# han0110/learn-fhe

Measured on AMD Instinct MI355X. Metric: NTTs/sec at N=2^14 q~60-bit, higher is better.
Workload: dtype u64

## Files before the change

learn-fhe_amd/csrc/arith.hpp:

```cpp
#pragma once
#include <type_traits>

#include "dev_arith.hpp"

namespace fhe {

#define FHE_GLOBAL __attribute__((address_space(1)))
template <class T>
__device__ __forceinline__ const FHE_GLOBAL T *as_global(const T *p) {
    return (const FHE_GLOBAL T *)p;
}
#define FHE_CONST __attribute__((address_space(4)))
template <class T>
__device__ __forceinline__ const FHE_CONST T *as_const(const T *p) {
    return (const FHE_CONST T *)p;
}

#define FHE_HEADER_KERNEL static __attribute__((unused)) __global__

template <int I, int END, typename F>
__device__ __forceinline__ void static_for(F &&f) {
    if constexpr (I < END) {
        f(std::integral_constant<int, I>{});
        static_for<I + 1, END>(f);
// ... 92 lines not shown
    static __device__ __forceinline__ u64 mac_in(u64 x, const K &k) { return canon4(x, k.q, k.q2); }
    static __device__ __forceinline__ u64 mac(u64 acc, u64 xin, u64 kval, int, const K &k, const Barrett &B) {
        return csub(acc + mulmod_barrett(xin, kval, B), k.q);
    }
    static __device__ __forceinline__ u64 mac_finish(u64 acc, const K &) { return acc; }
};

struct PmTw {
    unsigned wl, wlp, wh;
};
typedef uint2 PmRaw;
struct PmK {
    u64 q, q2, q4;
    unsigned c, c2;
};

__device__ __forceinline__ u64 mad_u64(unsigned a, unsigned b, u64 c) {
    u64 d, carry;
    asm("v_mad_u64_u32 %0, %1, %2, %3, %4" : "=v"(d), "=s"(carry) : "v"(a), "v"(b), "v"(c));
    return d;
}

__device__ __forceinline__ u64 hi_word(u64 x) {
    u64 d;
    asm("v_lshrrev_b64 %0, 32, %1" : "=v"(d) : "v"(x));
    return d;
}

template <int B>
__device__ __forceinline__ void pm_mul_vu(u64 y, const PmTw w, u64 &v, u64 &u) {
    const unsigned y0 = (unsigned)y, y1 = (unsigned)(y >> 32);
    const u64 z0 = (u64)w.wl * y0;
    const u64 z1 = (u64)w.wh * y0 + (u64)w.wlp * y1;
    v = mad_u64((unsigned)z1, 1u << (B - 31), z0);
    u = (u64)w.wh * y1 + hi_word(z1);
}

template <int B>
__device__ __forceinline__ u64 pm_reduce_vu(u64 v, u64 u, const PmK &k) {
    constexpr unsigned HMASK = (1u << (B - 32)) - 1;
    const u64 r1 = (u64)(unsigned)u * k.c2 + v;
    const u64 r2 = (u64)(unsigned)(u >> 32) * k.c2 + (r1 >> 32);
    const unsigned h2 = (unsigned)(r2 >> (B - 32));
    const u64 l2 = ((u64)((unsigned)r2 & HMASK) << 32) | (unsigned)r1;
    return (u64)h2 * k.c + l2;
}

template <int B>
__device__ __forceinline__ u64 pm_mul(u64 y, const PmTw w, const PmK &k) {
    u64 v, u;
    pm_mul_vu<B>(y, w, v, u);
    return pm_reduce_vu<B>(v, u, k);
}

template <int B>
struct ArithPM {
    typedef u64 Elem;
    static constexpr u64 MASK = (u64(1) << B) - 1;
    struct K {
        PmK m;
        const FHE_CONST PmRaw *tw, *twi;
        PmTw ninv;
        PmTw ninv_w;
        int pb, prefix;
    };
    typedef PmRaw TwRaw;
    typedef PmTw TwReg;
    static constexpr int PREFETCH = 4;
    static __host__ __device__ __forceinline__ u64 pack(u64 w) { return ((w >> (B - 31)) << 32) | (w & ((u64(1) << (B - 31)) - 1)); }
    template <bool INV>
    static __device__ __forceinline__ TwRaw fetch(const K &k, int idx) {
        const FHE_CONST PmRaw *p = (INV ? k.twi : k.tw) + idx;
        TwRaw r;
        r.x = p->x; r.y = p->y;
        return r;
    }
    static __device__ __forceinline__ TwReg prep(const TwRaw &r) { return PmTw{r.x, r.x << (63 - B), r.y}; }
    static __host__ __device__ __forceinline__ PmTw split(u64 w) {
        PmTw t;
        t.wl = (unsigned)(w & ((u64(1) << (B - 31)) - 1));
        t.wlp = t.wl << (63 - B);
        t.wh = (unsigned)(w >> (B - 31));
        return t;
    }
    static __device__ __forceinline__ K make(const ModDesc &D, int log_n_total, int pb, int prefix) {
        K k;
        k.m.q = D.q; k.m.q2 = 2 * D.q; k.m.q4 = 4 * D.q;
        k.m.c = D.pm_c; k.m.c2 = 2 * D.pm_c;
        k.tw = (const FHE_CONST PmRaw *)D.tww; k.twi = (const FHE_CONST PmRaw *)D.twwi;
        k.ninv = split(pb ? 1 : D.ninv[log_n_total]);
        k.ninv_w = split(D.ninv_w[log_n_total]);
        k.pb = pb; k.prefix = prefix;
        return k;
    }
    static __device__ __forceinline__ u64 fold1(u64 x, const PmK &m) {
        const unsigned hi = (unsigned)(x >> 32), h = hi >> (B - 32);
        const u64 base = ((u64)(hi & (unsigned)(MASK >> 32)) << 32) | (unsigned)x;
        return (u64)h * m.c + base;
    }
    static __device__ __forceinline__ u64 mulvar(u64 x, u64 y, const K &k) { return pm_mul<B>(x, split(y), k.m); }
    static __device__ __forceinline__ void ct(u64 &X, u64 &Y, const TwReg &w, const K &k) {
        const u64 t = pm_mul<B>(Y, w, k.m);
        const u64 x = X;
        X = x + t;
        Y = x - t + k.m.q2;
    }
    template <int PH>
    static __device__ __forceinline__ void gs(u64 &X, u64 &Y, const TwReg &w, const K &k) {
        const u64 s = X + Y;
        const u64 d = X - Y + (PH ? k.m.q4 : k.m.q2);
        X = s;
        Y = pm_mul<B>(d, w, k.m);
    }
    static constexpr bool GS_FOLDS = true;
    static constexpr int GS_SPAN = 0;
    template <int PH = 1>
    static __device__ __forceinline__ void gs_last_scaled(u64 &X, u64 &Y, const K &k) {
        const u64 s = X + Y, d = X - Y + k.m.q4;
        X = csub(pm_mul<B>(s, k.ninv, k.m), k.m.q);
        Y = csub(pm_mul<B>(d, k.ninv_w, k.m), k.m.q);
    }
    template <int PH = 1>
    static __device__ __forceinline__ void gs_last_plain(u64 &X, u64 &Y, const PmTw &w, const K &k) {
        const u64 s = X + Y, d = X - Y + k.m.q4;
        X = csub(fold1(s, k.m), k.m.q);
        Y = csub(pm_mul<B>(d, w, k.m), k.m.q);
    }
    static constexpr int CT_LAYERS = ((1 << (63 - B)) + 1) / 2 > 64 ? 64 : ((1 << (63 - B)) + 1) / 2;
    static constexpr bool PASS_FOLD = true;
    static __device__ constexpr bool ct_fold_at(int) { return false; }
    static __device__ __forceinline__ u64 gs_fold(u64 x, const K &k) { return fold1(x, k.m); }
    static __device__ __forceinline__ u64 fold(u64 x, const K &k) { return fold1(x, k.m); }
    static __device__ __forceinline__ u64 canon_fwd(u64 x, const K &k) { return csub(fold1(x, k.m), k.m.q); }
    static __device__ __forceinline__ u64 finish_inv(u64 x, const K &k) { return csub(pm_mul<B>(x, k.ninv, k.m), k.m.q); }
    static constexpr int MAC_TERMS = B <= 54 ? 32 : B == 55 ? 16 : B == 56 ? 8 : 3;
    struct MacAcc { u64 v, u; };
    static __device__ __forceinline__ MacAcc mac_zero() { return MacAcc{0, 0}; }
    static __device__ __forceinline__ u64 mac_in(u64 x, const K &) { return x; }
    static __device__ __forceinline__ MacAcc mac(MacAcc acc, u64 xin, u64 kval, int term, const K &k, const Barrett &) {
        const unsigned wl = (unsigned)kval;
        const PmTw w{wl, wl << (63 - B), (unsigned)(kval >> 32)};
        u64 v, u;
        pm_mul_vu<B>(xin, w, v, u);
        acc.v += v; acc.u += u;
        if ((term % MAC_TERMS) == MAC_TERMS - 1) acc = MacAcc{pm_reduce_vu<B>(acc.v, acc.u, k.m), 0};
        return acc;
    }
    static __device__ __forceinline__ u64 mac_finish(MacAcc acc, const K &k) { return pm_reduce_vu<B>(acc.v, acc.u, k.m); }
};

struct DsK {
    u64 q, q2, q4;
    unsigned c, c2, pw;
};

template <int B>
struct ArithDS {
    typedef u64 Elem;
    static constexpr u64 MASK = (u64(1) << B) - 1;
    static constexpr int SPLIT = B - 31;
    typedef uint4 TwRaw;
    typedef uint4 TwReg;
    struct K {
        DsK m;
        const FHE_CONST uint4 *tw, *twi;
        uint4 ninv, ninv_w;
        int pb, prefix;
        const FHE_CONST uint4 *tw3i;
        unsigned tw3_stride;
    };
    static constexpr int PREFETCH = 4;
    static __host__ __device__ __forceinline__ uint4 split(u64 w, u64 q) {
        const u64 w1 = (u64)((((unsigned __int128)w) << 32) % q);
        const u64 lo = (u64(1) << SPLIT) - 1;
        return uint4{(unsigned)(w & lo), (unsigned)(w >> SPLIT), (unsigned)(w1 & lo), (unsigned)(w1 >> SPLIT)};
    }
    template <bool INV>
    static __device__ __forceinline__ TwRaw fetch(const K &k, int idx) {
        const FHE_CONST uint4 *p = (INV ? k.twi : k.tw) + idx;
        TwRaw r;
        r.x = p->x; r.y = p->y; r.z = p->z; r.w = p->w;
        return r;
    }
    static __device__ __forceinline__ TwReg prep(const TwRaw &r) { return r; }
    static __device__ __forceinline__ K make(const ModDesc &D, int log_n_total, int pb, int prefix) {
        K k;
        k.m.q = D.q; k.m.q2 = 2 * D.q; k.m.q4 = 4 * D.q;
        k.m.c = D.pm_c; k.m.c2 = 2 * D.pm_c; k.m.pw = D.ds_pow;
        k.tw = as_const(D.twd); k.twi = as_const(D.twdi);
        k.ninv = pb ? D.ds_one : D.ds_ninv[log_n_total];
        k.ninv_w = D.ds_ninv_w[log_n_total];
        k.pb = pb; k.prefix = prefix;
        k.tw3i = as_const(D.twd3i); k.tw3_stride = D.twd3_stride;
        return k;
    }
    static __device__ __forceinline__ u64 mul_raw(u64 y, const uint4 &w, const DsK &m) {
        const unsigned y0 = (unsigned)y, y1 = (unsigned)(y >> 32);
        const u64 s1 = (u64)w.y * y0 + (u64)w.w * y1;
        const u64 s0 = (u64)w.x * y0 + (u64)w.z * y1;
        const u64 v = (u64)(unsigned)s1 * m.pw + s0;
        return (u64)(unsigned)(s1 >> 32) * m.c2 + v;
    }
    static __device__ __forceinline__ u64 fold1(u64 x, const DsK &m) {
        const unsigned hi = (unsigned)(x >> 32), h = hi >> (B - 32);
        const u64 base = ((u64)(hi & (unsigned)(MASK >> 32)) << 32) | (unsigned)x;
        return (u64)h * m.c + base;
    }
    static __device__ __forceinline__ u64 mul(u64 y, const uint4 &w, const DsK &m) { return fold1(mul_raw(y, w, m), m); }
    static __device__ __forceinline__ u64 mulvar(u64 x, u64 y, const K &k) {
        return pm_mul<B>(x, ArithPM<B>::split(y), PmK{k.m.q, k.m.q2, k.m.q4, k.m.c, k.m.c2});
    }
    static __device__ __forceinline__ void ct(u64 &X, u64 &Y, const TwReg &w, const K &k) {
        const u64 t = mul(Y, w, k.m);
        const u64 x = X;
        X = x + t;
        Y = x + k.m.q2 - t;
    }
    static constexpr int CT_LAYERS = 64;
    static constexpr bool PASS_FOLD = false;
    static constexpr int CT_SPAN = B >= 64 - 2 ? 1 : (((1 << (64 - B)) - 2) / 2 > 64 ? 64 : ((1 << (64 - B)) - 2) / 2);
    static __device__ constexpr bool ct_fold_at(int layer) { return layer > 0 && layer % CT_SPAN == 0; }
    template <int PH>
    static __device__ __forceinline__ void gs(u64 &X, u64 &Y, const TwReg &w, const K &k) {
        static_assert(PH < 64 - B - 1, "sums overflow");
        const u64 s = X + Y;
        const u64 d = X + (k.m.q2 << PH) - Y;
        X = s;
        Y = mul(d, w, k.m);
    }
    static constexpr bool GS_FOLDS = true;
    static constexpr int GS_SPAN = 64 - B - 1 > 8 ? 8 : 64 - B - 1;
    template <int PH = 1>
    static __device__ __forceinline__ void gs_last_scaled(u64 &X, u64 &Y, const K &k) {
        const u64 s = X + Y, d = X + (k.m.q2 << PH) - Y;
        X = csub(mul(s, k.ninv, k.m), k.m.q);
        Y = csub(mul(d, k.ninv_w, k.m), k.m.q);
    }
    template <int PH = 1>
    static __device__ __forceinline__ void gs_last_plain(u64 &X, u64 &Y, const TwReg &w, const K &k) {
        const u64 s = X + Y, d = X + (k.m.q2 << PH) - Y;
        X = csub(fold1(s, k.m), k.m.q);
        Y = csub(mul(d, w, k.m), k.m.q);
    }
    static __device__ __forceinline__ u64 gs_fold(u64 x, const K &k) { return fold1(x, k.m); }
    static __device__ __forceinline__ u64 fold(u64 x, const K &k) { return fold1(x, k.m); }
    static __device__ __forceinline__ u64 canon_fwd(u64 x, const K &k) { return csub(fold1(x, k.m), k.m.q); }
    static __device__ __forceinline__ u64 finish_inv(u64 x, const K &k) { return csub(mul(x, k.ninv, k.m), k.m.q); }
    typedef typename ArithPM<B>::MacAcc MacAcc;
    static constexpr int MAC_TERMS = ArithPM<B>::MAC_TERMS;
    static __device__ __forceinline__ PmK pmk(const K &k) { return PmK{k.m.q, k.m.q2, k.m.q4, k.m.c, k.m.c2}; }
    static __device__ __forceinline__ MacAcc mac_zero() { return MacAcc{0, 0}; }
    static __device__ __forceinline__ u64 mac_in(u64 x, const K &) { return x; }
    static __device__ __forceinline__ MacAcc mac(MacAcc acc, u64 xin, u64 kval, int term, const K &k, const Barrett &) {
        const unsigned wl = (unsigned)kval;
        const PmTw w{wl, wl << (63 - B), (unsigned)(kval >> 32)};
        u64 v, u;
        pm_mul_vu<B>(xin, w, v, u);
        acc.v += v; acc.u += u;
        if ((term % MAC_TERMS) == MAC_TERMS - 1) acc = MacAcc{pm_reduce_vu<B>(acc.v, acc.u, pmk(k)), 0};
        return acc;
    }
    static __device__ __forceinline__ u64 mac_finish(MacAcc acc, const K &k) { return pm_reduce_vu<B>(acc.v, acc.u, pmk(k)); }
};

#define FHE_SCHED_FENCE() asm volatile("" ::: "memory")

template <int L0_, int R_, int l_, int REP0_, int NREP_, int STRIDE_, bool SHARED_, int REP_SHIFT_ = 0>
struct Unit {
    static constexpr int L0 = L0_, R = R_, l = l_, REP0 = REP0_, NREP = NREP_, STRIDE = STRIDE_, REP_SHIFT = REP_SHIFT_;
    static constexpr bool SHARED = SHARED_;
    static constexpr int NT = (SHARED_ ? 1 : NREP_) << l_;
    static constexpr int half = 1 << (R_ - 1 - l_);
};

#ifdef FHE_LAB_ABLATE
template <class A, class = void> struct tw_skip_mask { static constexpr unsigned value = 0; };
template <class A> struct tw_skip_mask<A, decltype((void)A::SKIP_MASK)> { static constexpr unsigned value = A::SKIP_MASK; };
#endif

template <class A, bool INV, class U, int NTW>
__device__ __forceinline__ void tw_load(typename A::TwRaw (&raw)[NTW], int top, const typename A::K &k) {
    static_assert(U::NT <= NTW, "twiddle buffer too small for this unit");
#pragma unroll
    for (int rr = 0; rr < (U::SHARED ? 1 : U::NREP); ++rr)
#pragma unroll
        for (int b = 0; b < (1 << U::l); ++b) {
            const int tp = U::SHARED ? top : (top | ((U::REP0 + rr) << U::REP_SHIFT));
            const int idx = (1 << (U::L0 + U::l + k.pb)) + ((((k.prefix << U::L0) | tp)) << U::l) + b;
#ifdef FHE_LAB_ABLATE
            if constexpr ((tw_skip_mask<A>::value >> (U::L0 + U::l)) & 1) { raw[(rr << U::l) | b] = A::fake(k, idx); continue; }
#endif
            raw[(rr << U::l) | b] = A::template fetch<INV>(k, idx);
        }
}

template <class A, class U, int NTW, int E>
__device__ __forceinline__ void ct_apply(typename A::Elem (&x)[E], const typename A::TwRaw (&raw)[NTW], const typename A::K &k) {
    if constexpr ((U::l > 0 && U::l % A::CT_LAYERS == 0) || A::ct_fold_at(U::L0 + U::l)) {
#pragma unroll
        for (int rr = 0; rr < U::NREP; ++rr)
#pragma unroll
            for (int r = 0; r < (1 << U::R); ++r) x[(U::REP0 + rr) * U::STRIDE + r] = A::fold(x[(U::REP0 + rr) * U::STRIDE + r], k);
    }
    if constexpr (U::SHARED) {
#pragma unroll
        for (int b = 0; b < (1 << U::l); ++b) {
            const typename A::TwReg w = A::prep(raw[b]);
#pragma unroll
            for (int rr = 0; rr < U::NREP; ++rr)
#pragma unroll
                for (int j = 0; j < U::half; ++j) {
                    const int o = (U::REP0 + rr) * U::STRIDE + b * 2 * U::half + j;
                    A::ct(x[o], x[o + U::half], w, k);
                }
        }
    } else {
#pragma unroll
        for (int rr = 0; rr < U::NREP; ++rr)
#pragma unroll
            for (int b = 0; b < (1 << U::l); ++b) {
                const typename A::TwReg w = A::prep(raw[(rr << U::l) | b]);
#pragma unroll
                for (int j = 0; j < U::half; ++j) {
                    const int o = (U::REP0 + rr) * U::STRIDE + b * 2 * U::half + j;
                    A::ct(x[o], x[o + U::half], w, k);
                }
            }
    }
}

template <class A, class U, int GSTEP = -1, int NTW, int E>
__device__ __forceinline__ void gs_apply(typename A::Elem (&x)[E], const typename A::TwRaw (&raw)[NTW], const typename A::K &k) {
    constexpr bool GLOBAL = GSTEP >= 0 && A::GS_SPAN > 0;
    constexpr int step = U::R - 1 - U::l, PH = GLOBAL ? GSTEP % (A::GS_SPAN > 0 ? A::GS_SPAN : 1) : (step & 1);
    constexpr bool FOLD = A::GS_FOLDS && (GLOBAL ? PH == A::GS_SPAN - 1 : (PH == 1 || step == U::R - 1));
    static_for<0, (U::SHARED ? (1 << U::l) : U::NREP)>([&](auto oc) {
        constexpr int outer = decltype(oc)::value;
        static_for<0, (U::SHARED ? U::NREP : (1 << U::l))>([&](auto ic) {
            constexpr int inner = decltype(ic)::value;
            constexpr int b = U::SHARED ? outer : inner, rr = U::SHARED ? inner : outer;
            const typename A::TwReg w = A::prep(raw[U::SHARED ? b : ((rr << U::l) | b)]);
#pragma unroll
            for (int j = 0; j < U::half; ++j) {
                const int o = (U::REP0 + rr) * U::STRIDE + b * 2 * U::half + j;
                A::template gs<PH>(x[o], x[o + U::half], w, k);
                if constexpr (FOLD) x[o] = A::gs_fold(x[o], k);
            }
        });
    });
}

template <class A, int L0, int R, int OFF, int E>
__device__ __forceinline__ void ct_net(typename A::Elem (&x)[E], int top, const typename A::K &k) {
    static_for<0, R>([&](auto lc) {
        constexpr int l = decltype(lc)::value;
        typedef Unit<L0, R, l, 1, 1, OFF, true> U;
        if constexpr (l > 0) FHE_SCHED_FENCE();
        typename A::TwRaw raw[1 << l];
        tw_load<A, false, U>(raw, top, k);
        ct_apply<A, U>(x, raw, k);
    });
}

template <class A, int L0, int R, int OFF, int E>
__device__ __forceinline__ void gs_net(typename A::Elem (&x)[E], int top, const typename A::K &k) {
    static_for<0, R>([&](auto sc) {
        constexpr int l = R - 1 - decltype(sc)::value;
        typedef Unit<L0, R, l, 1, 1, OFF, true> U;
        if constexpr (l < R - 1) FHE_SCHED_FENCE();
        typename A::TwRaw raw[1 << l];
        tw_load<A, true, U>(raw, top, k);
        gs_apply<A, U>(x, raw, k);
    });
}

}
```

learn-fhe_amd/csrc/ntt14w.hpp:

```cpp
#pragma once
#include <type_traits>
#include "ntt_kernels.hpp"

namespace fhe {
namespace w14 {

constexpr int WSLOTS = 1088;
template <int R0> constexpr int threads() { return 64 << R0; }
template <int R0> constexpr size_t lds_bytes() { return (size_t(1) << R0) * WSLOTS * 8; }
constexpr int THREADS = threads<3>();
constexpr size_t LDS_BYTES = lds_bytes<3>();

__device__ __forceinline__ void wave_sync() {
    __builtin_amdgcn_wave_barrier();
    asm volatile("" ::: "memory");
}
#ifndef W14_XCHG_PRIO
#define W14_XCHG_PRIO 0
#endif
#if W14_XCHG_PRIO
#define W14_PRIO_UP() __builtin_amdgcn_s_setprio(3)
#define W14_PRIO_DOWN() __builtin_amdgcn_s_setprio(0)
#else
#define W14_PRIO_UP()
// ... 50 lines not shown
    u64 *wp = lds + (PAIRS ? 2 * t : t), *rp = lds + (w << 10) + (t & 63);
    u64 y[32];
    W14_PRIO_UP();
#pragma unroll
    for (int h = 0; h < 2; ++h) {
        if constexpr (PAIRS) {
#pragma unroll
            for (int lo = 0; lo < NLOW / 2; ++lo)
#pragma unroll
                for (int n = 0; n < (1 << R0); ++n) {
                    const int r = ((((h * (NLOW / 2)) | lo) << 1) << R0) | n;
                    *reinterpret_cast<ulonglong2 *>(wp + ((n << 10) | (lo << (7 + R0)))) = make_ulonglong2(x[r], x[r + (1 << R0)]);
                }
        } else {
#pragma unroll
            for (int lo = 0; lo < NLOW; ++lo)
#pragma unroll
                for (int n = 0; n < (1 << R0); ++n) wp[(n << 10) | (lo << (10 - (PB - 1)))] = x[((((h << (PB - 1)) | lo)) << R0) | n];
        }
        W14_SYNC();
#pragma unroll
        for (int m = 0; m < 16; ++m) {
            const int n4 = (h << 3) | (m >> 1), s = m & 1;
            y[(s << 4) | n4] = rp[m << 6];
        }
        W14_SYNC();
    }
    W14_PRIO_DOWN();
#pragma unroll
    for (int r = 0; r < 32; ++r) x[r] = y[r];
}

template <int R0, bool PAIRS>
__device__ __forceinline__ void xchg_10(u64 (&x)[32], int t, int w, u64 *lds) {
    constexpr int PB = 5 - R0, NLOW = 1 << (PB - 1);
    u64 *rp = lds + (PAIRS ? 2 * t : t), *wp = lds + (w << 10) + (t & 63);
    u64 y[32];
    W14_PRIO_UP();
    W14_SYNC();
#pragma unroll
    for (int h = 0; h < 2; ++h) {
#pragma unroll
        for (int m = 0; m < 16; ++m) {
            const int n4 = (h << 3) | (m >> 1), s = m & 1;
            wp[m << 6] = x[(s << 4) | n4];
        }
        W14_SYNC();
        if constexpr (PAIRS) {
#pragma unroll
            for (int lo = 0; lo < NLOW / 2; ++lo)
#pragma unroll
                for (int n = 0; n < (1 << R0); ++n) {
                    const int r = ((((h * (NLOW / 2)) | lo) << 1) << R0) | n;
                    const ulonglong2 v = *reinterpret_cast<const ulonglong2 *>(rp + ((n << 10) | (lo << (7 + R0))));
                    y[r] = v.x; y[r + (1 << R0)] = v.y;
                }
        } else {
#pragma unroll
            for (int lo = 0; lo < NLOW; ++lo)
#pragma unroll
                for (int n = 0; n < (1 << R0); ++n) y[((((h << (PB - 1)) | lo)) << R0) | n] = rp[(n << 10) | (lo << (10 - (PB - 1)))];
        }
        if (h == 0) W14_SYNC();
    }
    W14_PRIO_DOWN();
#pragma unroll
    for (int r = 0; r < 32; ++r) x[r] = y[r];
}

__device__ __forceinline__ void xchg_12(u64 (&x)[32], int lane, u64 *wl) {
    u64 *wp = wl + lane;
    const u64 *rp = wl + 68 * (lane >> 2) + (lane & 3);
    u64 y[32];
    W14_PRIO_UP();
#pragma unroll
    for (int h = 0; h < 2; ++h) {
#pragma unroll
        for (int n4 = 0; n4 < 16; ++n4) wp[68 * n4] = x[(h << 4) | n4];
        wave_sync();
#pragma unroll
        for (int r4 = 0; r4 < 16; ++r4)
            y[((r4 & 1) << 4) | (h << 3) | (r4 >> 1)] = rp[4 * r4];
        wave_sync();
    }
    W14_PRIO_DOWN();
#pragma unroll
    for (int r = 0; r < 32; ++r) x[r] = y[r];
}

__device__ __forceinline__ void xchg_21(u64 (&x)[32], int lane, u64 *wl) {
    u64 *wp = wl + 68 * (lane >> 2) + (lane & 3);
    const u64 *rp = wl + lane;
    u64 y[32];
    W14_PRIO_UP();
#pragma unroll
    for (int h = 0; h < 2; ++h) {
#pragma unroll
        for (int r4 = 0; r4 < 16; ++r4) wp[4 * r4] = x[((r4 & 1) << 4) | (h << 3) | (r4 >> 1)];
        wave_sync();
#pragma unroll
        for (int n4 = 0; n4 < 16; ++n4) y[(h << 4) | n4] = rp[68 * n4];
        wave_sync();
    }
    W14_PRIO_DOWN();
#pragma unroll
    for (int r = 0; r < 32; ++r) x[r] = y[r];
}

__device__ __forceinline__ void xchg_23(u64 (&x)[32], int lane, u64 *wl) {
    const int hi5 = ((lane >> 4) << 3) | ((lane & 3) << 1) | ((lane >> 3) & 1);
    u64 *wp = wl + 34 * hi5 + ((lane >> 2) & 1);
    const u64 *rp = wl + 34 * (lane >> 5) + 2 * (lane & 15) + ((lane >> 4) & 1);
    u64 y[32];
    W14_PRIO_UP();
#pragma unroll
    for (int h = 0; h < 2; ++h) {
#pragma unroll
        for (int c = 0; c < 16; ++c) wp[2 * c] = x[(h << 4) | c];
        wave_sync();
#pragma unroll
        for (int R = 0; R < 16; ++R)
            y[((R >> 2) << 3) | (h << 2) | (R & 3)] = rp[68 * R];
        wave_sync();
    }
    W14_PRIO_DOWN();
#pragma unroll
    for (int r = 0; r < 32; ++r) x[r] = y[r];
}

__device__ __forceinline__ void xchg_32(u64 (&x)[32], int lane, u64 *wl) {
    const u64 *rp = wl + 17 * lane;
    u64 *wp = wl + 68 * (lane >> 4) + (lane & 15);
    u64 y[32];
    W14_PRIO_UP();
#pragma unroll
    for (int h = 0; h < 2; ++h) {
#pragma unroll
        for (int R = 0; R < 16; ++R) wp[17 * (((R >> 2) << 4) | (R & 3))] = x[((R >> 2) << 3) | (h << 2) | (R & 3)];
        wave_sync();
#pragma unroll
        for (int c = 0; c < 16; ++c) y[(h << 4) | c] = rp[c];
        wave_sync();
    }
    W14_PRIO_DOWN();
#pragma unroll
    for (int r = 0; r < 32; ++r) x[r] = y[r];
}

template <int R0, int l> using P0 = Unit<0, R0, l, 0, (32 >> R0), (1 << R0), true>;
template <int R0, int l> using P1 = Unit<R0, 4, l, 0, 2, 16, true>;
template <int R0, int l> using P2 = Unit<R0 + 4, 4, l, 0, 2, 16, true>;
template <int R0, int l, int AB> using P3 = Unit<R0 + 8, 3, l, AB, 1, 8, false, 6>;

#ifndef W14_P3_REFILL
#define W14_P3_REFILL -1
#endif
template <class A>
__device__ __host__ constexpr bool w14_p3_refill() {
    return W14_P3_REFILL < 0 ? std::is_same<typename A::TwRaw, uint4>::value : W14_P3_REFILL != 0;
}

template <class A>
struct Tw7 {
    typename A::TwRaw l0[1], l1[2], l2[4];
};
template <class A, bool INV, int R0, int AB>
__device__ __forceinline__ void tw7_load(Tw7<A> &b, int t3, const typename A::K &k) {
    tw_load<A, INV, P3<R0, 0, AB>>(b.l0, t3, k);
    tw_load<A, INV, P3<R0, 1, AB>>(b.l1, t3, k);
    tw_load<A, INV, P3<R0, 2, AB>>(b.l2, t3, k);
}

template <int R0, bool PAIRS>
__device__ __forceinline__ void load_p0(u64 (&x)[32], const u64 *__restrict__ g, int t) {
#pragma unroll
    for (int r = 0; r < 32; ++r) {
        const int n = r & ((1 << R0) - 1), pass = r >> R0;
#ifdef W14_ABLATE_NO_GLOBAL
        x[r] = (u64)(t + r) * 0x9E3779B97F4A7C15ull >> 5;
#else
        if constexpr (PAIRS) {
            if (pass & 1) continue;
            const ulonglong2 v = *reinterpret_cast<const ulonglong2 *>(g + ((n << 11) | ((pass >> 1) << (7 + R0)) | (t << 1)));
            x[r] = v.x; x[r + (1 << R0)] = v.y;
        } else {
            x[r] = g[(n << 11) | (pass << (6 + R0)) | t];
        }
#endif
    }
}
template <int AB>
__device__ __forceinline__ void load_p3(u64 (&x)[32], const u64 *__restrict__ src) {
#pragma unroll
    for (int j = 0; j < 8; j += 2) {
        const ulonglong2 v = *reinterpret_cast<const ulonglong2 *>(src + (AB << 9) + j);
        x[AB * 8 + j] = v.x; x[AB * 8 + j + 1] = v.y;
    }
}
template <class A, int AB>
__device__ __forceinline__ void load_mul_p3(u64 (&x)[32], const u64 *__restrict__ src, const u64 *__restrict__ mul, const typename A::K &k) {
#pragma unroll
    for (int j = 0; j < 8; j += 2) {
        const ulonglong2 v = *reinterpret_cast<const ulonglong2 *>(src + (AB << 9) + j);
        const ulonglong2 m = *reinterpret_cast<const ulonglong2 *>(mul + (AB << 9) + j);
        x[AB * 8 + j] = A::mulvar(v.x, m.x, k); x[AB * 8 + j + 1] = A::mulvar(v.y, m.y, k);
    }
}

template <class A, int AB>
__device__ __forceinline__ void store_p3(u64 (&x)[32], u64 *__restrict__ dst_wave, int lane, u64 *wl, const typename A::K &k) {
    ulonglong2 *wr = reinterpret_cast<ulonglong2 *>(wl + 8 * lane + (lane & ~1));
    const ulonglong2 *rd = reinterpret_cast<const ulonglong2 *>(wl + 2 * lane + 2 * (lane >> 3));
#pragma unroll
    for (int j = 0; j < 4; ++j) {
        ulonglong2 v;
        v.x = A::canon_fwd(x[AB * 8 + 2 * j], k);
        v.y = A::canon_fwd(x[AB * 8 + 2 * j + 1], k);
        wr[j] = v;
    }
    wave_sync();
#pragma unroll
    for (int kk = 0; kk < 4; ++kk) {
        const ulonglong2 v = rd[72 * kk];
        x[AB * 8 + 2 * kk] = v.x; x[AB * 8 + 2 * kk + 1] = v.y;
    }
    wave_sync();
#pragma unroll
    for (int kk = 0; kk < 4; ++kk) {
        ulonglong2 v;
        v.x = x[AB * 8 + 2 * kk]; v.y = x[AB * 8 + 2 * kk + 1];
#ifdef W14_ABLATE_NO_GLOBAL
        if (v.x == 0xdeadbeefcafef00dull)
#endif
        *reinterpret_cast<ulonglong2 *>(dst_wave + (AB << 9) + 128 * kk + 2 * lane) = v;
    }
}

template <class A, int R0, bool KEEP = false>
__device__ __forceinline__ void fwd_one(u64 (&x)[32], u64 *__restrict__ g, const typename A::K &k, u64 *lds, u64 *wl,
                                        const int t, const int lane, const int w STAMP_ENTRY_PARAM) {
    typedef typename A::TwRaw Tw;
    STAMP_DECL;
    STAMP_REAL(10);
    STAMP(0);
    {
        Tw a0[1], a1[2], a2[4], a3[8];
        tw_load<A, false, P0<R0, 0>>(a0, 0, k);
        if constexpr (R0 >= 2) tw_load<A, false, P0<R0, (R0 >= 2 ? 1 : 0)>>(a1, 0, k);
        if constexpr (R0 >= 3) tw_load<A, false, P0<R0, (R0 >= 3 ? 2 : 0)>>(a2, 0, k);
        if constexpr (R0 == 4) tw_load<A, false, P0<R0, (R0 == 4 ? 3 : 0)>>(a3, 0, k);
        STAMP(1);
        FHE_SCHED_FENCE();
        ct_apply<A, P0<R0, 0>>(x, a0, k);
        if constexpr (R0 >= 2) {
            FHE_SCHED_FENCE();
            ct_apply<A, P0<R0, (R0 >= 2 ? 1 : 0)>>(x, a1, k);
        }
        if constexpr (R0 >= 3) {
            FHE_SCHED_FENCE();
            ct_apply<A, P0<R0, (R0 >= 3 ? 2 : 0)>>(x, a2, k);
        }
        if constexpr (R0 == 4) {
            FHE_SCHED_FENCE();
            ct_apply<A, P0<R0, (R0 == 4 ? 3 : 0)>>(x, a3, k);
        }
    }
    FHE_SCHED_FENCE();
    Tw b0[1], b1[2], b2[4], b3[8];
    tw_load<A, false, P1<R0, 0>>(b0, w, k); tw_load<A, false, P1<R0, 1>>(b1, w, k); tw_load<A, false, P1<R0, 2>>(b2, w, k); tw_load<A, false, P1<R0, 3>>(b3, w, k);
    STAMP(2);
    xchg_01<R0, w14_pairs<A, R0>()>(x, t, w, lds);
    STAMP(3);
    if constexpr (A::PASS_FOLD) {
#pragma unroll
        for (int r = 0; r < 32; ++r) x[r] = A::fold(x[r], k);
    }
    FHE_SCHED_FENCE();
    ct_apply<A, P1<R0, 0>>(x, b0, k);
    FHE_SCHED_FENCE();
    ct_apply<A, P1<R0, 1>>(x, b1, k);
    FHE_SCHED_FENCE();
    ct_apply<A, P1<R0, 2>>(x, b2, k);
    FHE_SCHED_FENCE();
    ct_apply<A, P1<R0, 3>>(x, b3, k);
    FHE_SCHED_FENCE();
    const int t2 = (w << 4) | (lane >> 2), t3 = (w << 8) | lane;
    Tw c0[1], c1[2], c2[4], c3[8];
    tw_load<A, false, P2<R0, 0>>(c0, t2, k); tw_load<A, false, P2<R0, 1>>(c1, t2, k); tw_load<A, false, P2<R0, 2>>(c2, t2, k);
    STAMP(4);
    xchg_12(x, lane, wl);
    STAMP(5);
    if constexpr (A::PASS_FOLD) {
#pragma unroll
        for (int r = 0; r < 32; ++r) x[r] = A::fold(x[r], k);
    }
    FHE_SCHED_FENCE();
    ct_apply<A, P2<R0, 0>>(x, c0, k);
    FHE_SCHED_FENCE();
    ct_apply<A, P2<R0, 1>>(x, c1, k);
    FHE_SCHED_FENCE();
    tw_load<A, false, P2<R0, 3>>(c3, t2, k);
    ct_apply<A, P2<R0, 2>>(x, c2, k);
    FHE_SCHED_FENCE();
    ct_apply<A, P2<R0, 3>>(x, c3, k);
    FHE_SCHED_FENCE();
    Tw7<A> d[2];
    tw7_load<A, false, R0, 0>(d[0], t3, k);
    STAMP(6);
    xchg_23(x, lane, wl);
    STAMP(7);
    if constexpr (A::PASS_FOLD) {
#pragma unroll
        for (int r = 0; r < 32; ++r) x[r] = A::fold(x[r], k);
    }
    u64 *dst_wave = g + (w << 11);
    static_for<0, 4>([&](auto abc) {
        constexpr int ab = decltype(abc)::value;
        FHE_SCHED_FENCE();
        ct_apply<A, P3<R0, 0, ab>>(x, d[ab & 1].l0, k);
        ct_apply<A, P3<R0, 1, ab>>(x, d[ab & 1].l1, k);
        FHE_SCHED_FENCE();
        if constexpr (ab < 3) tw7_load<A, false, R0, (ab < 3 ? ab + 1 : 3)>(d[(ab + 1) & 1], t3, k);
        ct_apply<A, P3<R0, 2, ab>>(x, d[ab & 1].l2, k);
        FHE_SCHED_FENCE();
        if constexpr (KEEP) {
#pragma unroll
            for (int j = 0; j < 8; ++j) x[ab * 8 + j] = A::canon_fwd(x[ab * 8 + j], k);
        } else {
            store_p3<A, ab>(x, dst_wave, lane, wl, k);
        }
    });
    STAMP(8);
#ifdef NTT14_STAMPS
    asm volatile("s_waitcnt vmcnt(0)" ::: "memory");
#endif
    STAMP(9);
    STAMP_REAL(11);
    STAMP_FLUSH();
}

template <class A>
__device__ __host__ constexpr bool w14_p3_diag() {
#ifdef W14_NO_DIAG
    return false;
#else
    return std::is_same<typename A::TwRaw, uint4>::value;
#endif
}

template <class A, int R0, int AB>
__device__ __forceinline__ int p3_blk(int t3, const typename A::K &k) {
    return (1 << (R0 + 8 + k.pb)) + ((k.prefix << (R0 + 8)) | t3 | (AB << 6));
}
template <class A, int R0, int AB>
__device__ __forceinline__ void p3_diag_load(uint4 (&e)[7], int t3, const typename A::K &k) {
    const int blk = p3_blk<A, R0, AB>(t3, k);
#pragma unroll
    for (int p = 0; p < 7; ++p) {
        const FHE_CONST uint4 *q = k.tw3i + size_t(p) * k.tw3_stride + blk;
        e[p] = uint4{q->x, q->y, q->z, q->w};
    }
}
template <class A, int R0, int AB, int NEXT>
__device__ __forceinline__ void p3_diag_apply(u64 (&x)[32], uint4 (&e)[7], const uint4 &ci, const uint4 &cj, const uint4 &cij, int t3,
                                              const typename A::K &k) {
    const auto &m = k.m;
    u64 *v = x + 8 * AB;
    const u64 s0 = v[0] + v[1], t0 = v[0] + m.q2 - v[1];
    const u64 s1 = v[2] + v[3], t1 = A::mul(v[2] + m.q2 - v[3], ci, m);
    const u64 s2 = v[4] + v[5], t2 = A::mul(v[4] + m.q2 - v[5], cj, m);
    const u64 s3 = v[6] + v[7], t3v = A::mul(v[6] + m.q2 - v[7], cij, m);
    const u64 u0 = s0 + s1, e0 = s0 + m.q4 - s1;
    const u64 u1 = t0 + t1, e1 = t0 + m.q2 - t1;
    const u64 u2 = s2 + s3, e2 = A::mul(s2 + m.q4 - s3, ci, m);
    const u64 u3 = t2 + t3v, e3 = A::mul(t2 + m.q2 - t3v, ci, m);
    const int blk = NEXT >= 0 ? p3_blk<A, R0, (NEXT >= 0 ? NEXT : 0)>(t3, k) : 0;
    auto refill = [&](int p) {
        if constexpr (NEXT >= 0) {
            const FHE_CONST uint4 *q = k.tw3i + size_t(p) * k.tw3_stride + blk;
            e[p] = uint4{q->x, q->y, q->z, q->w};
        }
    };
    v[0] = A::fold1(u0 + u2, m);
    v[1] = A::mul(u1 + u3, e[0], m); refill(0);
    v[2] = A::mul(e0 + e2, e[1], m); refill(1);
    v[3] = A::mul(e1 + e3, e[2], m); refill(2);
    v[4] = A::mul(u0 + m.q4 - u2, e[3], m); refill(3);
    v[5] = A::mul(u1 + m.q4 - u3, e[4], m); refill(4);
    v[6] = A::mul(e0 + m.q2 - e2, e[5], m); refill(5);
    v[7] = A::mul(e1 + m.q2 - e3, e[6], m); refill(6);
}

template <class A, bool PFX, int R0>
__device__ __forceinline__ void inv_one(u64 (&x)[32], Tw7<A> (&d)[2], u64 *__restrict__ g, const typename A::K &k, u64 *lds, u64 *wl,
                                        const int t, const int lane, const int w STAMP_ENTRY_PARAM) {
    typedef typename A::TwRaw Tw;
    const int t2 = (w << 4) | (lane >> 2), t3 = (w << 8) | lane;
    STAMP_DECL;
    STAMP_REAL(10);
    STAMP(0);
    constexpr bool REFILL = w14_p3_refill<A>();
    Tw c3[8], c2[4], c1[2], c0[1];
    if constexpr (w14_p3_diag<A>()) {
        uint4(&e)[7] = reinterpret_cast<uint4(&)[7]>(d[0]);
        const uint4 ci = A::template fetch<true>(k, 1), cj = A::template fetch<true>(k, 2), cij = A::template fetch<true>(k, 3);
        FHE_SCHED_FENCE();
        p3_diag_apply<A, R0, 0, 1>(x, e, ci, cj, cij, t3, k);
        FHE_SCHED_FENCE();
        p3_diag_apply<A, R0, 1, 2>(x, e, ci, cj, cij, t3, k);
        FHE_SCHED_FENCE();
        p3_diag_apply<A, R0, 2, 3>(x, e, ci, cj, cij, t3, k);
        FHE_SCHED_FENCE();
        p3_diag_apply<A, R0, 3, -1>(x, e, ci, cj, cij, t3, k);
    } else
    static_for<0, 4>([&](auto abc) {
        constexpr int ab = decltype(abc)::value, nx = ab < 3 ? ab + 1 : 3;
        Tw7<A> &e = d[REFILL ? 0 : ab & 1];
        FHE_SCHED_FENCE();
        gs_apply<A, P3<R0, 2, ab>, 0>(x, e.l2, k);
        if constexpr (REFILL && ab < 3) tw_load<A, true, P3<R0, 2, nx>>(e.l2, t3, k);
        FHE_SCHED_FENCE();
        gs_apply<A, P3<R0, 1, ab>, 1>(x, e.l1, k);
        if constexpr (REFILL && ab < 3) tw_load<A, true, P3<R0, 1, nx>>(e.l1, t3, k);
        gs_apply<A, P3<R0, 0, ab>, 2>(x, e.l0, k);
        if constexpr (REFILL && ab < 3) tw_load<A, true, P3<R0, 0, nx>>(e.l0, t3, k);
        FHE_SCHED_FENCE();
        if constexpr (!REFILL && ab < 2) tw7_load<A, true, R0, (ab < 2 ? ab + 2 : 3)>(d[ab & 1], t3, k);
    });
    FHE_SCHED_FENCE();
    STAMP(1);
    constexpr bool C3_LATE = sizeof(Tw) > 8;
    if constexpr (!C3_LATE) tw_load<A, true, P2<R0, 3>>(c3, t2, k);
    xchg_32(x, lane, wl);
    STAMP(2);
    FHE_SCHED_FENCE();
    if constexpr (C3_LATE) tw_load<A, true, P2<R0, 3>>(c3, t2, k);
    tw_load<A, true, P2<R0, 2>>(c2, t2, k);
    gs_apply<A, P2<R0, 3>, 3>(x, c3, k);
    FHE_SCHED_FENCE();
    tw_load<A, true, P2<R0, 1>>(c1, t2, k); tw_load<A, true, P2<R0, 0>>(c0, t2, k);
    gs_apply<A, P2<R0, 2>, 4>(x, c2, k);
    FHE_SCHED_FENCE();
    gs_apply<A, P2<R0, 1>, 5>(x, c1, k);
    FHE_SCHED_FENCE();
    gs_apply<A, P2<R0, 0>, 6>(x, c0, k);
    FHE_SCHED_FENCE();
    STAMP(3);
    Tw b3[8], b2[4], b1[2], b0[1];
    tw_load<A, true, P1<R0, 3>>(b3, w, k); tw_load<A, true, P1<R0, 2>>(b2, w, k); tw_load<A, true, P1<R0, 1>>(b1, w, k); tw_load<A, true, P1<R0, 0>>(b0, w, k);
    xchg_21(x, lane, wl);
    STAMP(4);
    FHE_SCHED_FENCE();
    gs_apply<A, P1<R0, 3>, 7>(x, b3, k);
    FHE_SCHED_FENCE();
    gs_apply<A, P1<R0, 2>, 8>(x, b2, k);
    FHE_SCHED_FENCE();
    gs_apply<A, P1<R0, 1>, 9>(x, b1, k);
    FHE_SCHED_FENCE();
    gs_apply<A, P1<R0, 0>, 10>(x, b0, k);
    FHE_SCHED_FENCE();
    STAMP(5);
    Tw a3[8], a2[4], a1[2], a0[1];
    if constexpr (R0 == 4) tw_load<A, true, P0<R0, (R0 == 4 ? 3 : 0)>>(a3, 0, k);
    if constexpr (R0 >= 3) tw_load<A, true, P0<R0, (R0 >= 3 ? 2 : 0)>>(a2, 0, k);
    if constexpr (R0 >= 2) tw_load<A, true, P0<R0, (R0 >= 2 ? 1 : 0)>>(a1, 0, k);
    if constexpr (PFX) tw_load<A, true, P0<R0, 0>>(a0, 0, k);
    xchg_10<R0, w14_pairs<A, R0>()>(x, t, w, lds);
    STAMP(6);
    if constexpr (R0 == 4) {
        FHE_SCHED_FENCE();
        gs_apply<A, P0<R0, (R0 == 4 ? 3 : 0)>, 11>(x, a3, k);
    }
    if constexpr (R0 >= 3) {
        FHE_SCHED_FENCE();
        gs_apply<A, P0<R0, (R0 >= 3 ? 2 : 0)>, 8 + R0>(x, a2, k);
    }
// ... 168 lines not shown
```

Measured before the change: 14.29 million.

## Schedule lazy reductions in forward NTT butterflies via compile-time overflow planner

Adds a compile-time schedule that tracks value bounds across forward NTT layers and decides per layer whether to skip the post-multiply fold (raw product with 8q offset) and where to fold only the X inputs. Butterflies whose output feeds the next layer's multiplicand take the raw path, which removes fold instructions from the hot loop. It is enabled for non-KEEP forward transforms, except R0=2 with 60-bit moduli. The risk is correctness near 64-bit overflow, guarded by static_asserts, plus some added template complexity.

New measurement: 14.53 million (median of 6 runs). +1.7%, better.

```diff
diff --git a/learn-fhe_amd/csrc/arith.hpp b/learn-fhe_amd/csrc/arith.hpp
--- a/learn-fhe_amd/csrc/arith.hpp
+++ b/learn-fhe_amd/csrc/arith.hpp
@@ -268,6 +268,58 @@
 struct DsK {
     u64 q, q2, q4;
     unsigned c, c2, pw;
+    u64 q8;
+};
+
+template <int LAYER_, int LAYERS_, int NEXT_>
+struct CtPos {
+    static constexpr int LAYER = LAYER_, LAYERS = LAYERS_, NEXT = NEXT_;
+};
+struct CtPlan {
+    bool fold_x, raw;
+};
+
+template <int B>
+struct DsCtSchedule {
+    typedef unsigned __int128 u128;
+    static constexpr u128 CMAX = u128(1) << (B - 33), TOP = u128(1) << 64;
+    static constexpr bool fits(int m, u128 e) { return (u128(m) << B) + e * CMAX <= TOP; }
+    static constexpr u128 FOLD_E = (u128(1) << (64 - B)) - 1;
+    static constexpr int RAW_OFFSET = 8;
+    static constexpr int gain_of_fold(int l, int n) {
+        int m = 1, g = 0;
+        for (int j = l; j < n && fits(m + RAW_OFFSET, FOLD_E); ++j, m += 2) g += j == n - 1 ? 16 : 8;
+        return g;
+    }
+    static constexpr CtPlan plan(int layer, int n) {
+        int m = 1;
+        u128 e = 0;
+        CtPlan p{false, false};
+        for (int l = 0; l <= layer; ++l) {
+            p.raw = fits(m + RAW_OFFSET, e);
+            p.fold_x = !p.raw && (gain_of_fold(l, n) > 16 || !fits(m + 2, e));
+            if (p.fold_x) {
+                m = 1; e = FOLD_E;
+                p.raw = fits(m + RAW_OFFSET, e);
+            }
+            m += 2;
+        }
+        return p;
+    }
+    static constexpr bool safe(int n) {
+        int m = 1;
+        u128 e = 0;
+        for (int l = 0; l < n; ++l) {
+            const CtPlan p = plan(l, n);
+            if (p.fold_x) { m = 1; e = FOLD_E; }
+            if (!fits(m + (p.raw ? RAW_OFFSET : 2), e)) return false;
+            m += 2;
+        }
+        return true;
+    }
+    static_assert(B >= 34 && B <= 60, "two-operand product: 34 <= B <= 60");
+    static_assert((u128(1) << 33) * CMAX <= (u128(1) << B) && 8 * CMAX < (u128(1) << B), "unfolded product exceeds its offset");
+    static_assert((FOLD_E + 2) * CMAX < (u128(1) << B), "a folded value does not canonicalise with one subtraction");
 };
 
 template <int B>
@@ -303,6 +355,7 @@
         K k;
         k.m.q = D.q; k.m.q2 = 2 * D.q; k.m.q4 = 4 * D.q;
         k.m.c = D.pm_c; k.m.c2 = 2 * D.pm_c; k.m.pw = D.ds_pow;
+        k.m.q8 = 8 * D.q;
         k.tw = as_const(D.twd); k.twi = as_const(D.twdi);
         k.ninv = pb ? D.ds_one : D.ds_ninv[log_n_total];
         k.ninv_w = D.ds_ninv_w[log_n_total];
@@ -332,6 +385,13 @@
         X = x + t;
         Y = x + k.m.q2 - t;
     }
+    static __device__ __forceinline__ void ct_raw(u64 &X, u64 &Y, const TwReg &w, const K &k) {
+        const u64 r = mul_raw(Y, w, k.m);
+        const u64 x = X;
+        X = x + r;
+        Y = x + k.m.q8 - r;
+    }
+    typedef DsCtSchedule<B> CtSchedule;
     static constexpr int CT_LAYERS = 64;
     static constexpr bool PASS_FOLD = false;
     static constexpr int CT_SPAN = B >= 64 - 2 ? 1 : (((1 << (64 - B)) - 2) / 2 > 64 ? 64 : ((1 << (64 - B)) - 2) / 2);
@@ -410,8 +470,37 @@
         }
 }
 
-template <class A, class U, int NTW, int E>
+template <class A, class = void> struct ct_schedule { typedef void type; };
+template <class A> struct ct_schedule<A, std::void_t<typename A::CtSchedule>> { typedef typename A::CtSchedule type; };
+
+template <class A, class U, class POS = void, int NTW, int E>
 __device__ __forceinline__ void ct_apply(typename A::Elem (&x)[E], const typename A::TwRaw (&raw)[NTW], const typename A::K &k) {
+    typedef typename ct_schedule<A>::type S;
+    if constexpr (!std::is_void<POS>::value && !std::is_void<S>::value) {
+        static_assert(S::safe(POS::LAYERS), "forward schedule overflows 64 bits");
+        static_assert(POS::NEXT == 0 ? POS::LAYER == POS::LAYERS - 1 : (POS::NEXT != U::half && POS::NEXT < E), "next layer's register bit");
+        constexpr CtPlan plan = S::plan(POS::LAYER, POS::LAYERS);
+        if constexpr (plan.fold_x) {
+            static_for<0, U::NREP << U::R>([&](auto rc) {
+                constexpr int r = (U::REP0 + (decltype(rc)::value >> U::R)) * U::STRIDE + (decltype(rc)::value & ((1 << U::R) - 1));
+                if constexpr ((r & U::half) == 0) x[r] = A::fold(x[r], k);
+            });
+        }
+        static_for<0, (U::SHARED ? (1 << U::l) : U::NREP)>([&](auto oc) {
+            constexpr int outer = decltype(oc)::value;
+            static_for<0, (U::SHARED ? U::NREP : (1 << U::l))>([&](auto ic) {
+                constexpr int inner = decltype(ic)::value;
+                constexpr int b = U::SHARED ? outer : inner, rr = U::SHARED ? inner : outer;
+                const typename A::TwReg w = A::prep(raw[U::SHARED ? b : ((rr << U::l) | b)]);
+                static_for<0, U::half>([&](auto jc) {
+                    constexpr int o = (U::REP0 + rr) * U::STRIDE + b * 2 * U::half + decltype(jc)::value;
+                    if constexpr (plan.raw && (POS::NEXT == 0 || (o & POS::NEXT) != 0)) A::ct_raw(x[o], x[o + U::half], w, k);
+                    else A::ct(x[o], x[o + U::half], w, k);
+                });
+            });
+        });
+        return;
+    }
     if constexpr ((U::l > 0 && U::l % A::CT_LAYERS == 0) || A::ct_fold_at(U::L0 + U::l)) {
 #pragma unroll
         for (int rr = 0; rr < U::NREP; ++rr)
diff --git a/learn-fhe_amd/csrc/ntt14w.hpp b/learn-fhe_amd/csrc/ntt14w.hpp
--- a/learn-fhe_amd/csrc/ntt14w.hpp
+++ b/learn-fhe_amd/csrc/ntt14w.hpp
@@ -226,6 +226,18 @@
 template <int R0, int l> using P2 = Unit<R0 + 4, 4, l, 0, 2, 16, true>;
 template <int R0, int l, int AB> using P3 = Unit<R0 + 8, 3, l, AB, 1, 8, false, 6>;
 
+template <int R0, class U>
+using FwdPos = CtPos<U::L0 + U::l, 11 + R0, (U::L0 + U::l == 10 + R0 ? 0 : U::l < U::R - 1 ? U::half / 2 : 16)>;
+template <class A, int R0, bool KEEP>
+__device__ __host__ constexpr bool w14_fwd_pos() {
+    return !KEEP && !(R0 == 2 && std::is_same<A, ArithDS<60>>::value);
+}
+template <class A, int R0, bool KEEP, class U, int NTW>
+__device__ __forceinline__ void ct_at(u64 (&x)[32], const typename A::TwRaw (&raw)[NTW], const typename A::K &k) {
+    if constexpr (w14_fwd_pos<A, R0, KEEP>()) ct_apply<A, U, FwdPos<R0, U>>(x, raw, k);
+    else ct_apply<A, U>(x, raw, k);
+}
+
 #ifndef W14_P3_REFILL
 #define W14_P3_REFILL -1
 #endif
@@ -325,18 +337,18 @@
         if constexpr (R0 == 4) tw_load<A, false, P0<R0, (R0 == 4 ? 3 : 0)>>(a3, 0, k);
         STAMP(1);
         FHE_SCHED_FENCE();
-        ct_apply<A, P0<R0, 0>>(x, a0, k);
+        ct_at<A, R0, KEEP, P0<R0, 0>>(x, a0, k);
         if constexpr (R0 >= 2) {
             FHE_SCHED_FENCE();
-            ct_apply<A, P0<R0, (R0 >= 2 ? 1 : 0)>>(x, a1, k);
+            ct_at<A, R0, KEEP, P0<R0, (R0 >= 2 ? 1 : 0)>>(x, a1, k);
         }
         if constexpr (R0 >= 3) {
             FHE_SCHED_FENCE();
-            ct_apply<A, P0<R0, (R0 >= 3 ? 2 : 0)>>(x, a2, k);
+            ct_at<A, R0, KEEP, P0<R0, (R0 >= 3 ? 2 : 0)>>(x, a2, k);
         }
         if constexpr (R0 == 4) {
             FHE_SCHED_FENCE();
-            ct_apply<A, P0<R0, (R0 == 4 ? 3 : 0)>>(x, a3, k);
+            ct_at<A, R0, KEEP, P0<R0, (R0 == 4 ? 3 : 0)>>(x, a3, k);
         }
     }
     FHE_SCHED_FENCE();
@@ -350,13 +362,13 @@
         for (int r = 0; r < 32; ++r) x[r] = A::fold(x[r], k);
     }
     FHE_SCHED_FENCE();
-    ct_apply<A, P1<R0, 0>>(x, b0, k);
-    FHE_SCHED_FENCE();
-    ct_apply<A, P1<R0, 1>>(x, b1, k);
-    FHE_SCHED_FENCE();
-    ct_apply<A, P1<R0, 2>>(x, b2, k);
-    FHE_SCHED_FENCE();
-    ct_apply<A, P1<R0, 3>>(x, b3, k);
+    ct_at<A, R0, KEEP, P1<R0, 0>>(x, b0, k);
+    FHE_SCHED_FENCE();
+    ct_at<A, R0, KEEP, P1<R0, 1>>(x, b1, k);
+    FHE_SCHED_FENCE();
+    ct_at<A, R0, KEEP, P1<R0, 2>>(x, b2, k);
+    FHE_SCHED_FENCE();
+    ct_at<A, R0, KEEP, P1<R0, 3>>(x, b3, k);
     FHE_SCHED_FENCE();
     const int t2 = (w << 4) | (lane >> 2), t3 = (w << 8) | lane;
     Tw c0[1], c1[2], c2[4], c3[8];
@@ -369,14 +381,14 @@
         for (int r = 0; r < 32; ++r) x[r] = A::fold(x[r], k);
     }
     FHE_SCHED_FENCE();
-    ct_apply<A, P2<R0, 0>>(x, c0, k);
-    FHE_SCHED_FENCE();
-    ct_apply<A, P2<R0, 1>>(x, c1, k);
+    ct_at<A, R0, KEEP, P2<R0, 0>>(x, c0, k);
+    FHE_SCHED_FENCE();
+    ct_at<A, R0, KEEP, P2<R0, 1>>(x, c1, k);
     FHE_SCHED_FENCE();
     tw_load<A, false, P2<R0, 3>>(c3, t2, k);
-    ct_apply<A, P2<R0, 2>>(x, c2, k);
-    FHE_SCHED_FENCE();
-    ct_apply<A, P2<R0, 3>>(x, c3, k);
+    ct_at<A, R0, KEEP, P2<R0, 2>>(x, c2, k);
+    FHE_SCHED_FENCE();
+    ct_at<A, R0, KEEP, P2<R0, 3>>(x, c3, k);
     FHE_SCHED_FENCE();
     Tw7<A> d[2];
     tw7_load<A, false, R0, 0>(d[0], t3, k);
@@ -391,11 +403,11 @@
     static_for<0, 4>([&](auto abc) {
         constexpr int ab = decltype(abc)::value;
         FHE_SCHED_FENCE();
-        ct_apply<A, P3<R0, 0, ab>>(x, d[ab & 1].l0, k);
-        ct_apply<A, P3<R0, 1, ab>>(x, d[ab & 1].l1, k);
+        ct_at<A, R0, KEEP, P3<R0, 0, ab>>(x, d[ab & 1].l0, k);
+        ct_at<A, R0, KEEP, P3<R0, 1, ab>>(x, d[ab & 1].l1, k);
         FHE_SCHED_FENCE();
         if constexpr (ab < 3) tw7_load<A, false, R0, (ab < 3 ? ab + 1 : 3)>(d[(ab + 1) & 1], t3, k);
-        ct_apply<A, P3<R0, 2, ab>>(x, d[ab & 1].l2, k);
+        ct_at<A, R0, KEEP, P3<R0, 2, ab>>(x, d[ab & 1].l2, k);
         FHE_SCHED_FENCE();
         if constexpr (KEEP) {
 #pragma unroll
```
